# jankammeth/BA-path-planning

Measured on AMD Instinct MI355X. Metric: SCP iterations/sec (N agents x K waypoints), higher is better.
Workload: dtype f64

## Files before the change

ba-path-planning_amd/csrc/scp_kernels.hip:

```cpp
#include "scp_common.h"
#include "scp_pair_device.h"

#include <sys/prctl.h>
#include <time.h>

#include <atomic>
#include <chrono>
#include <cmath>
#include <cstdlib>
#include <map>
#include <mutex>
#include <type_traits>
#include <utility>

extern "C" int scp_abi_version(void) { return SCP_ABI_VERSION; }

extern "C" int scp_ctx_create(int device, void* hip_stream, scp_ctx** out) {
  if (!out) return SCP_ERR_INVALID;
  *out = nullptr;
  if (hipSetDevice(device) != hipSuccess) return SCP_ERR_HIP;
  scp_ctx* ctx = new scp_ctx();
  memset(ctx, 0, sizeof(*ctx));
  ctx->device = device;
  ctx->stream = (hipStream_t)hip_stream;
// ... 1511 lines not shown
  }
  __syncthreads();
  *total = tot;
  return base + incl - v;
}

__global__ __launch_bounds__(CMP_THREADS) void compact_count_kernel(const uint32_t* __restrict__ map, int64_t words,
                                                                     uint32_t* __restrict__ block_tot) {
  const int64_t w0 = (int64_t)blockIdx.x * CMP_WORDS + (int64_t)threadIdx.x * CMP_WPT;
  int c = 0;
#pragma unroll
  for (int i = 0; i < CMP_WPT; ++i)
    if (w0 + i < words) c += __popc(map[w0 + i]);
  int tot;
  block_exclusive_scan(c, &tot);
  if (threadIdx.x == 0) block_tot[blockIdx.x] = (uint32_t)tot;
}

__device__ inline void publish_stats(const scp_pair_stats* stats, unsigned long long n_selected, scp_stats_mirror* mirror,
                                     unsigned long long seq) {
  if (!mirror) return;
  const double mind = __hip_atomic_load(&stats->min_dist, __ATOMIC_RELAXED, __HIP_MEMORY_SCOPE_AGENT);
  const double maxv = __hip_atomic_load(&stats->max_violation, __ATOMIC_RELAXED, __HIP_MEMORY_SCOPE_AGENT);
  const unsigned long long fv =
      __hip_atomic_load((const unsigned long long*)&stats->first_violation, __ATOMIC_RELAXED, __HIP_MEMORY_SCOPE_AGENT);
  __hip_atomic_store((unsigned long long*)&mirror->stats.min_dist, (unsigned long long)__double_as_longlong(mind),
                     __ATOMIC_RELAXED, __HIP_MEMORY_SCOPE_SYSTEM);
  __hip_atomic_store((unsigned long long*)&mirror->stats.first_violation, fv, __ATOMIC_RELAXED, __HIP_MEMORY_SCOPE_SYSTEM);
  __hip_atomic_store((unsigned long long*)&mirror->stats.n_selected, n_selected, __ATOMIC_RELAXED, __HIP_MEMORY_SCOPE_SYSTEM);
  __hip_atomic_store((unsigned long long*)&mirror->stats.max_violation, (unsigned long long)__double_as_longlong(maxv),
                     __ATOMIC_RELAXED, __HIP_MEMORY_SCOPE_SYSTEM);
  __hip_atomic_store((unsigned long long*)&mirror->seq, seq, __ATOMIC_RELEASE, __HIP_MEMORY_SCOPE_SYSTEM);
}

__global__ __launch_bounds__(CMP_THREADS) void compact_scan_kernel(uint32_t* __restrict__ block_tot, int nblocks,
                                                                    scp_pair_stats* __restrict__ stats,
                                                                    scp_stats_mirror* __restrict__ mirror,
                                                                    unsigned long long seq) {
  int carry = 0;
  for (int b0 = 0; b0 < nblocks; b0 += CMP_THREADS) {
    const int b = b0 + threadIdx.x;
    const int v = b < nblocks ? (int)block_tot[b] : 0;
    int tot;
    const int ex = block_exclusive_scan(v, &tot);
    if (b < nblocks) block_tot[b] = (uint32_t)(carry + ex);
    carry += tot;
  }
  if (threadIdx.x == 0) {
    stats->n_selected = (unsigned long long)carry;
    publish_stats(stats, (unsigned long long)carry, mirror, seq);
  }
}

__global__ __launch_bounds__(CMP_THREADS) void compact_write_kernel(uint32_t* __restrict__ map, int64_t words,
                                                                     const uint32_t* __restrict__ block_off, int64_t nq,
                                                                     int64_t q_begin, int64_t pairs,
                                                                     int64_t* __restrict__ rows, int64_t cap,
                                                                     uint32_t* __restrict__ merge_into,
                                                                     const scp_pair_stats* __restrict__ stats) {
  const bool overflow = merge_into != nullptr && stats->n_selected > (unsigned long long)cap;
  const int64_t w0 = (int64_t)blockIdx.x * CMP_WORDS + (int64_t)threadIdx.x * CMP_WPT;
  uint32_t wd[CMP_WPT];
  int c = 0;
#pragma unroll
  for (int i = 0; i < CMP_WPT; ++i) {
    wd[i] = (w0 + i < words) ? map[w0 + i] : 0u;
    c += __popc(wd[i]);
  }
  int tot;
  int64_t slot = (int64_t)block_off[blockIdx.x] + block_exclusive_scan(c, &tot);
  if (tot == 0) return;
#pragma unroll
  for (int i = 0; i < CMP_WPT; ++i) {
    uint32_t m = wd[i];
    if (m && merge_into) {
      if (!overflow) merge_into[w0 + i] |= m;
      map[w0 + i] = 0u;
    }
    if (m) {
      const int64_t base = (w0 + i) * 32;
      const int64_t kk = base / nq, rr = base - kk * nq;
      while (m) {
        const int bit = __ffs((int)m) - 1;
        m &= m - 1;
        int64_t k2 = kk, r2 = rr + bit;
        while (r2 >= nq) {
          r2 -= nq;
          ++k2;
        }
        if (!overflow && slot < cap) rows[slot] = k2 * pairs + q_begin + r2;
        ++slot;
      }
    }
  }
}

constexpr int CMP1_THREADS = 1024;

template <int THREADS, bool COHERENT>
__device__ inline int compact_small_body(uint32_t* __restrict__ map, int64_t words, int64_t nq, int64_t q_begin,
                                         int64_t pairs, int64_t* __restrict__ rows, int64_t cap,
                                         uint32_t* __restrict__ merge_into, bool overwrite) {
  __shared__ int wsum[THREADS / 64];
  __shared__ int total_sh;
  constexpr int CHUNK = THREADS * CMP_WPT;
  const int lane = threadIdx.x & 63, wave = threadIdx.x >> 6;
  auto load = [&](int64_t w) -> uint32_t {
    return COHERENT ? __hip_atomic_load(map + w, __ATOMIC_RELAXED, __HIP_MEMORY_SCOPE_AGENT) : map[w];
  };
  int c_all = 0;
  for (int64_t w = threadIdx.x; w < words; w += THREADS) c_all += __popc(load(w));
#pragma unroll
  for (int o = 32; o > 0; o >>= 1) c_all += __shfl_xor(c_all, o);
  __syncthreads();
  if (lane == 0) wsum[wave] = c_all;
  __syncthreads();
  if (threadIdx.x == 0) {
    int t = 0;
    for (int w = 0; w < THREADS / 64; ++w) t += wsum[w];
    total_sh = t;
  }
  __syncthreads();
  const int total = total_sh;
// ... 61 lines not shown
__global__ __launch_bounds__(CMP1_THREADS) void compact_small_kernel(uint32_t* __restrict__ map, int64_t words, int64_t nq,
                                                                      int64_t q_begin, int64_t pairs,
                                                                      int64_t* __restrict__ rows, int64_t cap,
                                                                      uint32_t* __restrict__ merge_into,
                                                                      scp_pair_stats* __restrict__ stats,
                                                                      scp_stats_mirror* __restrict__ mirror,
                                                                      unsigned long long seq) {
  const int total = compact_small_body<CMP1_THREADS, false>(map, words, nq, q_begin, pairs, rows, cap, merge_into, false);
  if (threadIdx.x == 0) {
    stats->n_selected = (unsigned long long)total;
    publish_stats(stats, (unsigned long long)total, mirror, seq);
  }
}

static int ensure_cmp(scp_ctx* ctx, int64_t words) {
  const size_t need_map = (size_t)words * sizeof(uint32_t);
  const size_t need_tot = (size_t)(scp_cdiv(words, CMP_WORDS) + 1) * sizeof(uint32_t);
  if (ctx->cmp_map_bytes < need_map) {
    if (ctx->cmp_map) {
      SCP_HIP_CHECK(ctx, hipStreamSynchronize(ctx->stream));
      SCP_HIP_CHECK(ctx, hipFree(ctx->cmp_map));
      ctx->cmp_map = nullptr;
      ctx->cmp_map_bytes = 0;
    }
    SCP_HIP_CHECK(ctx, hipMalloc(&ctx->cmp_map, need_map));
    SCP_HIP_CHECK(ctx, hipMemsetAsync(ctx->cmp_map, 0, need_map, ctx->stream));
    ctx->cmp_map_bytes = need_map;
  }
  if (ctx->cmp_tot_bytes < need_tot) {
    if (ctx->cmp_tot) {
      SCP_HIP_CHECK(ctx, hipStreamSynchronize(ctx->stream));
      SCP_HIP_CHECK(ctx, hipFree(ctx->cmp_tot));
      ctx->cmp_tot = nullptr;
      ctx->cmp_tot_bytes = 0;
    }
    SCP_HIP_CHECK(ctx, hipMalloc(&ctx->cmp_tot, need_tot));
    ctx->cmp_tot_bytes = need_tot;
  }
  return SCP_OK;
}

static int launch_compaction(scp_ctx* ctx, uint32_t* map, int64_t words, int64_t nq, int64_t q_begin, int64_t pairs,
                             int64_t* rows, int64_t cap, uint32_t* merge_into, scp_pair_stats* stats) {
  if (words <= 0) return SCP_OK;
  const unsigned long long seq = ++ctx->mirror_seq;
  if (words <= CMP1_MAX_WORDS) {
    hipLaunchKernelGGL(compact_small_kernel, dim3(1), dim3(CMP1_THREADS), 0, ctx->stream, map, words, nq, q_begin, pairs,
                       rows, cap, merge_into, stats, ctx->d_mirror, seq);
    SCP_HIP_CHECK(ctx, hipGetLastError());
    return SCP_OK;
  }
  const int nblocks = scp_cdiv(words, CMP_WORDS);
  hipLaunchKernelGGL(compact_count_kernel, dim3(nblocks), dim3(CMP_THREADS), 0, ctx->stream, map, words, ctx->cmp_tot);
  hipLaunchKernelGGL(compact_scan_kernel, dim3(1), dim3(CMP_THREADS), 0, ctx->stream, ctx->cmp_tot, nblocks, stats,
                     ctx->d_mirror, seq);
  hipLaunchKernelGGL(compact_write_kernel, dim3(nblocks), dim3(CMP_THREADS), 0, ctx->stream, map, words, ctx->cmp_tot,
                     nq, q_begin, pairs, rows, cap, merge_into, stats);
  SCP_HIP_CHECK(ctx, hipGetLastError());
  return SCP_OK;
}

static int check_pair_range(scp_ctx* ctx, int N, int K, int D, int64_t q_begin, int64_t q_end) {
  SCP_REQUIRE(ctx, N >= 1 && K >= 1 && (D == 2 || D == 3), "pair pass: bad shape N=%d K=%d D=%d", N, K, D);
  SCP_REQUIRE(ctx, q_begin >= 0 && q_end >= q_begin && q_end <= scp_pairs(N),
              "pair pass: bad pair range [%lld, %lld) of %lld", (long long)q_begin, (long long)q_end,
              (long long)scp_pairs(N));
  SCP_REQUIRE(ctx, K <= 65535, "pair pass: K=%d exceeds grid.y", K);
  SCP_REQUIRE(ctx, q_end - q_begin < ((int64_t)1 << 31) - 2 * PAIR_ROWS,
              "pair pass: %lld pairs per call exceed the 32-bit lane offsets; shard the pair range",
              (long long)(q_end - q_begin));
  return SCP_OK;
}

int scp_check_pair_range(scp_ctx* ctx, int N, int K, int D, int64_t q_begin, int64_t q_end) {
  return check_pair_range(ctx, N, K, D, q_begin, q_end);
}

extern "C" int scp_linearize_pairs(scp_ctx* ctx, int N, int K, int D, double R, double h, int64_t q_begin,
                                   int64_t q_end, const double* pos_prev, const double* p0, const double* v0,
                                   double* eta_out, double* l_out, double margin, int64_t* sel_rows,
                                   int64_t sel_cap, uint32_t* sel_bitmap, scp_pair_stats* stats) {
  if (!ctx) return SCP_ERR_INVALID;
  int rc = check_pair_range(ctx, N, K, D, q_begin, q_end);
  if (rc) return rc;
  SCP_REQUIRE(ctx, pos_prev && p0 && v0 && eta_out && l_out && sel_bitmap && stats && (sel_rows || sel_cap == 0),
              "linearize_pairs: null pointer");
  SCP_REQUIRE(ctx, ((uintptr_t)eta_out % 16 == 0) && ((uintptr_t)l_out % 16 == 0),
              "linearize_pairs: eta/l must be 16-byte aligned");
  const int64_t nq = q_end - q_begin;
  PairArgs a{};
  a.N = N; a.K = K; a.D = D; a.R = R; a.h = h;
  a.q_begin = q_begin; a.q_end = q_end; a.pairs = scp_pairs(N);
  a.eta = eta_out; a.l = l_out; a.margin = margin;
  a.bitmap = sel_bitmap; a.mark = sel_bitmap; a.stats = stats;
  a.eta_stride = scp_eta_stride(K, nq);
  const int64_t words = (K * nq + 31) / 32;
  rc = ensure_cmp(ctx, words);
  if (rc) return rc;
  rc = launch_pair_pass<MODE_LINEARIZE>(ctx, a, pos_prev, p0, v0, sel_bitmap, words);
  if (rc) return rc;
  return launch_compaction(ctx, sel_bitmap, words, nq, q_begin, a.pairs, sel_rows, sel_cap, nullptr, stats);
}

extern "C" int scp_select_pairs(scp_ctx* ctx, int N, int K, int D, double R, int64_t q_begin, int64_t q_end,
                                const double* pos_prev, double margin, int64_t* sel_rows, int64_t sel_cap,
                                uint32_t* sel_bitmap, scp_pair_stats* stats) {
  if (!ctx) return SCP_ERR_INVALID;
  int rc = check_pair_range(ctx, N, K, D, q_begin, q_end);
  if (rc) return rc;
  SCP_REQUIRE(ctx, pos_prev && sel_bitmap && stats && (sel_rows || sel_cap == 0), "select_pairs: null pointer");
// ... 253 lines not shown
```

ba-path-planning_amd/csrc/scp_qp_fused.hip:

```cpp
#include "scp_qp_device.h"
#include "scp_pair_device.h"
#include "scp_reset_device.h"
#include <cstdlib>

namespace {

using namespace scpdev;
constexpr int FT = 1024;
constexpr int NWV = FT / 64;

#ifdef SCP_PHASE_PROFILE
__device__ unsigned long long scp_phase_clk[64];
#define PHASE_MARK(slot)                                                                      \
  do {                                                                                        \
    if (blockIdx.x == gridDim.x / 2 && threadIdx.x == 0) scp_phase_clk[slot] = wall_clock64(); \
  } while (0)
#else
#define PHASE_MARK(slot) ((void)0)
#endif

constexpr int SQ_BLOCKS = 128;
template <int E>
__global__ __launch_bounds__(FT) void cg1_col_kernel(int K, int Rf, int64_t C, double rho, double h,
                                                      const double* __restrict__ pMinv, const double* __restrict__ wrow,
// ... 539 lines not shown
        const int64_t g = (int64_t)row * C + col;
        const double zh = alpha * fma(a, v1[u], v0[u]) + (1.0 - alpha) * v2[u];
        const double y = v3[u];
        const double zn = fmin(fmax(zh + y / rr[u], v4[u]), v5[u]);
        const double yn = y + rr[u] * (zh - zn);
        yf[g] = yn;
        zf[g] = zn;
        Fx[g] = fma(aa, v1[u], v0[u]);
        if (dyf) dyf[g] = yn - y;
      } else if (row < rows) {
        const int64_t g = (int64_t)(row - Rf) * C + col;
        x[g] = fma(aa, v1[u], v0[u]);
        Qn[g] = fma(aa, v3[u], v2[u]);
      }
    }
    return;
  }
  const int64_t n = (int64_t)(blockIdx.x - eblocks) * 256 + threadIdx.x;
  const bool live = n < nW;
  double e[D], qi[D], qj[D], pi[D], pj[D], z = 0.0, y = 0.0, lo = 0.0;
  int posi = 0, posj = 0;
  if (live) {
    const int64_t bi = (int64_t)wk[n] * C + (int64_t)wi[n] * D;
    const int64_t bj = (int64_t)wk[n] * C + (int64_t)wj[n] * D;
#pragma unroll
    for (int d = 0; d < D; ++d) {
      e[d] = weta[n * D + d];
      qi[d] = Qx[bi + d]; qj[d] = Qx[bj + d]; pi[d] = Qp[bi + d]; pj[d] = Qp[bj + d];
    }
    z = zc[n]; y = yc[n]; lo = wl[n];
    posi = pos_i[n]; posj = pos_j[n];
  }
  const double a = inline_sq ? step_length_inline_256<D>(part_rz, npart, nW, C, rho_c, wk, wi, wj, weta, Qp)
                             : step_length_256(part_rz, npart, part_sq);
  const double aa = alpha * a;
  if (!live) return;
  double tc = 0.0, ax = 0.0;
#pragma unroll
  for (int d = 0; d < D; ++d) {
    tc += e[d] * (fma(a, pi[d], qi[d]) - fma(a, pj[d], qj[d]));
    ax += e[d] * (fma(aa, pi[d], qi[d]) - fma(aa, pj[d], qj[d]));
  }
  const double zh = alpha * tc + (1.0 - alpha) * z;
  const double zn = fmax(zh + y / rho_c, lo);
  const double yn = y + rho_c * (zh - zn);
  yc[n] = yn;
  zc[n] = zn;
  if (dyc) dyc[n] = fmin(yn - y, 0.0);
  const double g = (rho_c * zn - yn) - rho_c * ax;
  gval[posi] = g;
  gval[posj] = g;
}

template <int D, bool INIT>
__global__ __launch_bounds__(256) void rows_value_kernel(int64_t nW, int64_t C, double rho, const int* __restrict__ wk,
                                                          const int* __restrict__ wi, const int* __restrict__ wj,
                                                          const double* __restrict__ weta, const double* __restrict__ Q,
                                                          const double* __restrict__ zc, const double* __restrict__ yc,
                                                          const int* __restrict__ pos_i, const int* __restrict__ pos_j,
                                                          double* __restrict__ gval) {
  const int64_t n = (int64_t)blockIdx.x * 256 + threadIdx.x;
  if (n >= nW) return;
  const int64_t bi = (int64_t)wk[n] * C + (int64_t)wi[n] * D;
  const int64_t bj = (int64_t)wk[n] * C + (int64_t)wj[n] * D;
  double ax = 0.0;
#pragma unroll
  for (int d = 0; d < D; ++d) ax += weta[n * D + d] * (Q[bi + d] - Q[bj + d]);
  const double g = INIT ? (rho * zc[n] - yc[n]) - rho * ax : rho * ax;
  gval[pos_i[n]] = g;
  gval[pos_j[n]] = g;
}

#define FUSED_LAUNCHED(qp) SCP_HIP_CHECK((qp)->ctx, hipGetLastError())

template <typename Kern>
int allow_lds(scp_qp* qp, Kern kernel, size_t bytes) {
  if (bytes <= 64 * 1024) return SCP_OK;
  SCP_HIP_CHECK(qp->ctx, scp_raise_lds_limit(qp->ctx->device, reinterpret_cast<const void*>(kernel), bytes));
  return SCP_OK;
}

}

int scp_qp_qp0_iterations(scp_qp* qp, int nit, double* dy_out) {
  const QpDev& d = qp->d;
  hipStream_t s = qp->ctx->stream;
  const int K = qp->K, Rf = qp->Rf;
  const int64_t C = qp->C;
  const int nblk = (int)((C + CB - 1) / CB);
  const size_t lds = (size_t)CB * (pad_col(Rf) + 3 * pad_col(K)) * sizeof(double);
  if (K <= 64) {
    int rc = allow_lds(qp, qp0_col_kernel<1>, lds);
    if (rc) return rc;
    hipLaunchKernelGGL(qp0_col_kernel<1>, dim3(nblk), dim3(FT), lds, s, K, Rf, C, qp->rho, qp->st.sigma, qp->st.alpha, qp->h,
                       nit, d.pMinv, d.wrow, d.lf, d.uf, d.x, d.zf, d.yf, dy_out);
  } else {
    int rc = allow_lds(qp, qp0_col_kernel<2>, lds);
    if (rc) return rc;
    hipLaunchKernelGGL(qp0_col_kernel<2>, dim3(nblk), dim3(FT), lds, s, K, Rf, C, qp->rho, qp->st.sigma, qp->st.alpha, qp->h,
                       nit, d.pMinv, d.wrow, d.lf, d.uf, d.x, d.zf, d.yf, dy_out);
  }
  FUSED_LAUNCHED(qp);
  return SCP_OK;
}

namespace {
constexpr int CSR1_MAX_CELLS = 16384;
constexpr int64_t CSR1_MAX_ROWS = 1 << 18;
struct CsrNewRows {
  int64_t n, base;
  const int64_t* rows;
  const double *pos_prev, *p0, *v0;
  double R, h;
  int N;
  int64_t* w_row;
  double* wl;
};
__global__ void csr_small_kernel(int64_t nW, int K, int ncell, int D, int64_t C, double rho, int* __restrict__ wk,
                                 int* __restrict__ wi, int* __restrict__ wj, double* __restrict__ weta,
                                 const double* __restrict__ Qx, double* __restrict__ zc, double* __restrict__ yc,
                                 int* __restrict__ ptr, int* __restrict__ ent, double* __restrict__ coef,
                                 int* __restrict__ pos_i, int* __restrict__ pos_j, double* __restrict__ gval, CsrNewRows nr);
}

int scp_qp_cg1_prepare(scp_qp* qp) {
  if (qp->dv.carried) return SCP_OK;
  const QpDev& d = qp->d;
  hipStream_t s = qp->ctx->stream;
  const int K = qp->K;
  const int64_t C = qp->C;
  const double rho_c = qp->rho * qp->st.rho_col_scale;
  QP_CHECK(scp_qp_exact_qx(qp, true));
  const double* Qx = scp_qp_qx(qp);
  if (qp->dv.vals_rho_c == rho_c) {
  } else if (!qp->dv.lists && qp->nW > 0 && qp->nW <= CSR1_MAX_ROWS && qp->N * K <= CSR1_MAX_CELLS) {
    const int ncell = qp->N * K;
    hipLaunchKernelGGL(csr_small_kernel, dim3(1), dim3(1024), (size_t)ncell * sizeof(int), s, qp->nW, K, ncell, qp->D, C, rho_c,
                       d.w_k, d.w_i, d.w_j, d.w_eta, Qx, d.zc, d.yc, d.cell_ptr, d.ent_code, d.coef, d.pos_i, d.pos_j, d.gval,
                       CsrNewRows{});
    FUSED_LAUNCHED(qp);
  } else {
    QP_CHECK(scp_qp_csr_ensure(qp));
    const dim3 rgrid((unsigned)((qp->nW + 255) / 256)), rblock(256);
    if (qp->D == 2)
      hipLaunchKernelGGL((rows_value_kernel<2, true>), rgrid, rblock, 0, s, qp->nW, C, rho_c, d.w_k, d.w_i, d.w_j, d.w_eta, Qx,
                         d.zc, d.yc, d.pos_i, d.pos_j, d.gval);
    else
      hipLaunchKernelGGL((rows_value_kernel<3, true>), rgrid, rblock, 0, s, qp->nW, C, rho_c, d.w_k, d.w_i, d.w_j, d.w_eta, Qx,
                         d.zc, d.yc, d.pos_i, d.pos_j, d.gval);
    FUSED_LAUNCHED(qp);
  }
  qp_on_cg1_prepared(qp);
  return SCP_OK;
}

int scp_qp_install_rows_small(scp_qp* qp, int64_t n, const int64_t* rows, const double* pos_prev, const double* p0,
                              const double* v0, double R, const double* Qx, bool* done) {
  *done = false;
  const QpDev& d = qp->d;
  const int K = qp->K;
  const int64_t nW = qp->nW + n;
  if (!qp->dv.qx || n <= 0 || nW > CSR1_MAX_ROWS || qp->N * K > CSR1_MAX_CELLS) return SCP_OK;
  const int ncell = qp->N * K;
  const double rho_c = qp->rho * qp->st.rho_col_scale;
  CsrNewRows nr{n, qp->nW, rows, pos_prev, p0, v0, R, qp->h, qp->N, d.w_row, d.w_l};
  hipLaunchKernelGGL(csr_small_kernel, dim3(1), dim3(1024), (size_t)ncell * sizeof(int), qp->ctx->stream, nW, K, ncell, qp->D,
                     qp->C, rho_c, d.w_k, d.w_i, d.w_j, d.w_eta, Qx, d.zc, d.yc, d.cell_ptr, d.ent_code, d.coef, d.pos_i,
                     d.pos_j, d.gval, nr);
  FUSED_LAUNCHED(qp);
  *done = true;
  return SCP_OK;
}

int scp_qp_cg1_iteration(scp_qp* qp, int* cg_count, bool emit_dy) {
  const QpDev& d = qp->d;
  double* dyf = emit_dy ? d.dyf : nullptr;
  double* dyc = emit_dy ? d.dyc : nullptr;
  hipStream_t s = qp->ctx->stream;
  const int K = qp->K, Rf = qp->Rf;
  const int64_t C = qp->C;
  const int nblk = (int)((C + CB - 1) / CB);
  double* Qp = d.s0p;
  double* Fp = d.tf;
  double* part_rz = d.part;
  double* part_sq = d.part + SCP_PART_CAP / 2;
  const double rho_c = qp->rho * qp->st.rho_col_scale;
  QP_CHECK(scp_qp_cg1_prepare(qp));
  double* Qx = scp_qp_qx(qp);
  double* Qn = scp_qp_qx(qp, true);
  const size_t lds = (size_t)CB * (pad_col(Rf) + 5 * pad_col(K)) * sizeof(double);
  int npart = nblk;
  if (K > SCP_FUSED_MAX_K) {
    npart = (int)C;
// ... 88 lines not shown

__global__ __launch_bounds__(256) void csr_scan_add_kernel(int ncell, int nblk, int* __restrict__ ptr, int* __restrict__ cur,
                                                            const int* __restrict__ blk_tot) {
  int off = 0;
  for (int b = 0; b < (int)blockIdx.x; ++b) off += blk_tot[b];
  const int c = blockIdx.x * SCAN_CELLS + SCAN_SC * (int)threadIdx.x;
#pragma unroll
  for (int e = 0; e < SCAN_SC; ++e) {
    if (c + e < ncell) {
      const int v = ptr[c + e] + off;
      ptr[c + e] = v;
      cur[c + e] = v;
    }
  }
  if (blockIdx.x == nblk - 1 && threadIdx.x == 0) ptr[ncell] = off + blk_tot[nblk - 1];
}

__global__ __launch_bounds__(256) void csr_fill_kernel(int64_t nW, int K, const int* __restrict__ wk,
                                                        const int* __restrict__ wi, const int* __restrict__ wj,
                                                        int* __restrict__ cur, int* __restrict__ ent) {
  const int64_t n = (int64_t)blockIdx.x * 256 + threadIdx.x;
  if (n >= nW) return;
  ent[atomicAdd(cur + cell_of(wk[n], wi[n], K), 1)] = (int)(2 * n);
  ent[atomicAdd(cur + cell_of(wk[n], wj[n], K), 1)] = (int)(2 * n + 1);
}

__global__ __launch_bounds__(256) void csr_sort_kernel(int ncell, const int* __restrict__ ptr, int* __restrict__ ent) {
  const int c = blockIdx.x * 256 + threadIdx.x;
  if (c >= ncell) return;
  const int b = ptr[c], e = ptr[c + 1];
  for (int i = b + 1; i < e; ++i) {
    const int v = ent[i];
    int j = i - 1;
    while (j >= b && ent[j] > v) {
      ent[j + 1] = ent[j];
      --j;
    }
    ent[j + 1] = v;
  }
}

__global__ __launch_bounds__(256) void csr_finish_kernel(int64_t nent, int D, const int* __restrict__ ent,
                                                          const double* __restrict__ weta, double* __restrict__ coef,
                                                          int* __restrict__ pos_i, int* __restrict__ pos_j) {
  const int64_t t = (int64_t)blockIdx.x * 256 + threadIdx.x;
  if (t >= nent) return;
  const int code = ent[t];
  const int n = code >> 1, side = code & 1;
  for (int d = 0; d < D; ++d) coef[t * D + d] = side ? -weta[(int64_t)n * D + d] : weta[(int64_t)n * D + d];
  if (side) pos_j[n] = (int)t;
  else pos_i[n] = (int)t;
}

template <bool COH>
__device__ inline void csr_small_body(int* csr_cnt, int64_t nW, int K, int ncell, int D, int64_t C, double rho,
                                                          int* __restrict__ wk, int* __restrict__ wi,
                                                          int* __restrict__ wj, double* __restrict__ weta,
                                                          const double* __restrict__ Qx, double* __restrict__ zc,
                                                          double* __restrict__ yc, int* __restrict__ ptr,
                                                          int* __restrict__ ent, double* __restrict__ coef,
                                                          int* __restrict__ pos_i, int* __restrict__ pos_j,
                                                          double* __restrict__ gval, CsrNewRows nr) {
  __shared__ int wsum[16];
  constexpr int SC = CSR1_MAX_CELLS / 1024;
  const int tid = threadIdx.x, lane = tid & 63, wave = tid >> 6;
  if (nr.n > 0) {
    const int64_t pairs = (int64_t)nr.N * (nr.N - 1) / 2;
    for (int64_t t = tid; t < nr.n; t += 1024) {
      if (D == 2)
        add_row_at<2, COH>(t, nr.N, K, C, pairs, nr.base, nr.rows, nr.pos_prev, nr.p0, nr.v0, nr.R, nr.h, Qx, nr.w_row, wk, wi, wj,
                      weta, nr.wl, zc, yc);
      else
        add_row_at<3, COH>(t, nr.N, K, C, pairs, nr.base, nr.rows, nr.pos_prev, nr.p0, nr.v0, nr.R, nr.h, Qx, nr.w_row, wk, wi, wj,
                      weta, nr.wl, zc, yc);
    }
    __threadfence_block();
    __syncthreads();
  }
  for (int c = tid; c < ncell; c += 1024) csr_cnt[c] = 0;
  __syncthreads();
  for (int64_t n = tid; n < nW; n += 1024) {
    atomicAdd(&csr_cnt[cell_of(wk[n], wi[n], K)], 1);
    atomicAdd(&csr_cnt[cell_of(wk[n], wj[n], K)], 1);
  }
  __syncthreads();
  {
    int v[SC], tot = 0;
#pragma unroll
    for (int e = 0; e < SC; ++e) {
      v[e] = SC * tid + e < ncell ? csr_cnt[SC * tid + e] : 0;
      tot += v[e];
    }
    int incl = tot;
#pragma unroll
    for (int o = 1; o < 64; o <<= 1) {
      const int t = __shfl_up(incl, o);
      if (lane >= o) incl += t;
    }
    if (lane == 63) wsum[wave] = incl;
    __syncthreads();
    int run = incl - tot;
    for (int w = 0; w < wave; ++w) run += wsum[w];
#pragma unroll
    for (int e = 0; e < SC; ++e) {
      if (SC * tid + e < ncell) {
        csr_cnt[SC * tid + e] = run;
// ... 88 lines not shown
                               const double* p0, const double* v0, double R, double* Qx, bool* done) {
  *done = false;
  const QpDev& d = qp->d;
  const int K = qp->K;
  if (n <= 0 || n > CSR1_MAX_ROWS || qp->N * K > CSR1_MAX_CELLS) return SCP_OK;
  const int ncell = qp->N * K;
  const double rho_c = qp->rho * qp->st.rho_col_scale;
  const size_t lds = std::max((size_t)K * RESET_COLS * sizeof(double), (size_t)ncell * sizeof(int));
  CsrNewRows nr{n, 0, rows, pos_prev, p0, v0, R, qp->h, qp->N, d.w_row, d.w_l};
  ResetArgs ra{qp->N, qp->Rf, x0, d.F, d.S0, d.x, d.zf, d.fx, d.yf};
  hipLaunchKernelGGL(reset_install_kernel, dim3((unsigned)scp_cdiv(qp->C, RESET_COLS)), dim3(1024), lds, qp->ctx->stream, ra, n,
                     K, ncell, qp->D, qp->C, rho_c, d.w_k, d.w_i, d.w_j, d.w_eta, Qx, d.zc, d.yc, d.cell_ptr, d.ent_code,
                     d.coef, d.pos_i, d.pos_j, d.gval, nr, qp->ctx->d_ticket + 2);
  FUSED_LAUNCHED(qp);
  *done = true;
  return SCP_OK;
}

namespace {
__global__ __launch_bounds__(256) void csr_rowval_kernel(int64_t nW, int mode, double rho, const double* __restrict__ zc,
                                                          const double* __restrict__ yc, const double* __restrict__ vec,
                                                          const int* __restrict__ pos_i, const int* __restrict__ pos_j,
                                                          double* __restrict__ gval, const double* __restrict__ vec2,
                                                          double* __restrict__ gval2) {
  const int64_t n = (int64_t)blockIdx.x * 256 + threadIdx.x;
  if (n >= nW) return;
  if (gval2) {
    const double g2 = vec2[n];
    gval2[pos_i[n]] = g2;
    gval2[pos_j[n]] = g2;
  }
  const double g = mode == 0 ? rho * zc[n] - yc[n] : (mode == 1 ? yc[n] : vec[n]);
  gval[pos_i[n]] = g;
  gval[pos_j[n]] = g;
}

__global__ __launch_bounds__(256) void csr_gather_kernel(int K, int N, int D, const int* __restrict__ ptr,
                                                          const double* __restrict__ coef,
                                                          const double* __restrict__ gval, double* __restrict__ G) {
  const int64_t t = (int64_t)blockIdx.x * 256 + threadIdx.x;
  const int64_t C = (int64_t)N * D;
  if (t >= C * K) return;
  const int k = (int)(t / C), col = (int)(t % C);
  const int agent = col / D, d = col - agent * D;
  const int cell = cell_of(k, agent, K);
  double acc = 0.0;
  const int t1 = ptr[cell + 1];
  for (int e = ptr[cell]; e < t1; ++e) acc += coef[(size_t)e * D + d] * gval[e];
  G[t] = acc;
}

}

int scp_qp_csr_ensure(scp_qp* qp) {
  if (qp->dv.lists) return SCP_OK;
  const QpDev& d = qp->d;
  hipStream_t s = qp->ctx->stream;
  const int ncell = qp->N * qp->K;
  SCP_REQUIRE(qp->ctx, 2 * qp->nW < 0x3FFFFFFF, "csr_build: too many working rows for 32-bit entry codes");
  SCP_HIP_CHECK(qp->ctx, hipMemsetAsync(d.cell_ptr, 0, (size_t)(ncell + 1) * sizeof(int), s));
  if (qp->nW > 0) {
    const dim3 rgrid((unsigned)((qp->nW + 255) / 256));
    hipLaunchKernelGGL(csr_count_kernel, rgrid, dim3(256), 0, s, qp->nW, qp->K, d.w_k, d.w_i, d.w_j, d.cell_ptr);
    const int sblk = (ncell + SCAN_CELLS - 1) / SCAN_CELLS;
    hipLaunchKernelGGL(csr_scan_local_kernel, dim3(sblk), dim3(256), 0, s, ncell, d.cell_ptr, d.scan_tot);
    hipLaunchKernelGGL(csr_scan_add_kernel, dim3(sblk), dim3(256), 0, s, ncell, sblk, d.cell_ptr, d.cell_cur, d.scan_tot);
    hipLaunchKernelGGL(csr_fill_kernel, rgrid, dim3(256), 0, s, qp->nW, qp->K, d.w_k, d.w_i, d.w_j, d.cell_cur, d.ent_code);
    hipLaunchKernelGGL(csr_sort_kernel, dim3((ncell + 255) / 256), dim3(256), 0, s, ncell, d.cell_ptr, d.ent_code);
    hipLaunchKernelGGL(csr_finish_kernel, dim3((unsigned)((2 * qp->nW + 255) / 256)), dim3(256), 0, s, 2 * qp->nW, qp->D,
                       d.ent_code, d.w_eta, d.coef, d.pos_i, d.pos_j);
    FUSED_LAUNCHED(qp);
  }
  qp_on_lists_built(qp);
  return SCP_OK;
}

int scp_qp_csr_scatter(scp_qp* qp, int mode, const double* vec) {
  QP_CHECK(scp_qp_csr_ensure(qp));
  const QpDev& d = qp->d;
  hipStream_t s = qp->ctx->stream;
  const int64_t nx = (int64_t)qp->K * qp->C;
  hipLaunchKernelGGL(csr_rowval_kernel, dim3((unsigned)((qp->nW + 255) / 256)), dim3(256), 0, s, qp->nW, mode,
                     qp->rho * qp->st.rho_col_scale, d.zc, d.yc, vec, d.pos_i, d.pos_j, d.gval, (const double*)nullptr, (double*)nullptr);
  hipLaunchKernelGGL(csr_gather_kernel, dim3((unsigned)((nx + 255) / 256)), dim3(256), 0, s, qp->K, qp->N, qp->D,
                     d.cell_ptr, d.coef, d.gval, d.G);
  FUSED_LAUNCHED(qp);
  return SCP_OK;
}

int scp_qp_rows_gather(scp_qp* qp, const double* Q) {
  const QpDev& d = qp->d;
  hipStream_t s = qp->ctx->stream;
  QP_CHECK(scp_qp_csr_ensure(qp));
  const int64_t C = qp->C, nx = (int64_t)qp->K * C;
  const double rho_c = qp->rho * qp->st.rho_col_scale;
  const dim3 rgrid((unsigned)((qp->nW + 255) / 256)), rblock(256);
  if (qp->D == 2)
    hipLaunchKernelGGL((rows_value_kernel<2, false>), rgrid, rblock, 0, s, qp->nW, C, rho_c, d.w_k, d.w_i, d.w_j, d.w_eta, Q,
                       d.zc, d.yc, d.pos_i, d.pos_j, d.gval);
  else
    hipLaunchKernelGGL((rows_value_kernel<3, false>), rgrid, rblock, 0, s, qp->nW, C, rho_c, d.w_k, d.w_i, d.w_j, d.w_eta, Q,
                       d.zc, d.yc, d.pos_i, d.pos_j, d.gval);
  hipLaunchKernelGGL(csr_gather_kernel, dim3((unsigned)((nx + 255) / 256)), dim3(256), 0, s, qp->K, qp->N, qp->D,
                     d.cell_ptr, d.coef, d.gval, d.G);
  FUSED_LAUNCHED(qp);
  return SCP_OK;
}

namespace {
struct PackDesc {
  const double* src;
  double* dst;
  int R, M;
};
struct PackArgs {
  PackDesc m[2];
};
__global__ __launch_bounds__(256) void pack_operands_kernel(PackArgs a) {
  const PackDesc d = a.m[blockIdx.y];
  const int nks = (d.M + 3) >> 2;
// ... 328 lines not shown
```

ba-path-planning_amd/csrc/scp_qp_internal.h:

```cpp
#pragma once
#include "scp_common.h"

constexpr int SCP_KKT_SLOTS = 6;
constexpr int SCP_KKT_SLOTS_MAX = 32;
constexpr size_t SCP_KKT_POOL_BYTES = (size_t)48 << 20;
constexpr int NPART = 128;

#define QP_CHECK(call)            \
  do {                            \
    int rc_ = (call);             \
    if (rc_ != SCP_OK) return rc_; \
  } while (0)

enum Slot {
  SL_RZ0 = 0, SL_RZ1 = 1,
  SL_RP = 8, SL_NAX = 9, SL_NZ = 10, SL_RD = 11, SL_NPX = 12, SL_NATY = 13,
  SL_NDY = 14, SL_SUPP = 15, SL_NATDY = 16,
  SL_COUNT = 32
};

struct QpDev {
  double *F, *Ft, *S0, *S0t, *HS, *Hf, *Minv, *aug, *wrow;
  double* gj_tmp;
  double* G0;
  double* pMinv;
  double *T, *pT;
  double *lf, *uf, *zf, *yf, *wf, *tf;
  double* states;
  double *x, *xt, *rhs, *r, *p, *zz, *G;
  double* HQ;
  int64_t* w_row;
  int *w_k, *w_i, *w_j;
  double *w_eta, *w_l, *zc, *yc;
  double* scal;
  double* part;
  double* s0p;
  double* fx;
  double* dyf;
  double* dyc;
  int* cell_ptr;
  int* cell_cur;
  int* scan_tot;
  int* ent_code;
  double* coef;
  double* gval;
  double* gval2;
  double* gval3;
  int *pos_i, *pos_j;
  double* kkt_pool;
  unsigned long long* sync_words;
  unsigned long long* cells;
  unsigned long long* gpart;
  unsigned long long* gcheck;
};

struct QpDerived {
  bool lists = false;
  bool qx = false;
  int qx_half = 0;
  double vals_rho_c = 0.0;
  bool carried = false;
};

struct scp_qp {
  scp_ctx* ctx;
  int N, K, D, Rf;
  int64_t C;
  double h;
  scp_qp_settings st;
  int64_t row_cap, nW;
  bool problem_set, reset_done;
  QpDerived dv;
  double rho;
  QpDev d;
  struct KktSlot {
    double rho, sigma;
    unsigned long long used;
    double *Hf, *HS, *Minv, *T, *pMinv, *pT;
  } kkt[SCP_KKT_SLOTS_MAX];
  int n_kkt;
  unsigned long long kkt_clock;
  double* h_scal;
  double* h_scal_dev;
  unsigned long long check_seq;
  double space[6];
  double lim[6];
  int64_t steps_since_reset;
  int persist_variant;
  int persist_fault;
  bool persist_off;
  bool persist_skip_solve;
  int persist_gave_up_total;
  int64_t persist_cap_nW;
  int persist_cap;
  unsigned long long persist_epoch;
  unsigned* h_persist;
  int persist_rho_switches;
  double persist_rho;
  unsigned* h_persist_dev;
};

constexpr int64_t SCP_FINE_MAX_COLUMNS = 4096;
inline int scp_qp_fine_cadence(const scp_qp* qp) {
  const scp_qp_settings& st = qp->st;
  const bool fine = st.check_fine > 0 && st.check_fine < st.check_termination && st.check_termination % st.check_fine == 0 &&
                    qp->nW > 0 && qp->C <= SCP_FINE_MAX_COLUMNS;
  return fine ? st.check_fine : 0;
}

constexpr int SCP_RESID_STRIDE = 12;
constexpr int SCP_RESID_CAP = (4096 / 2 + 128) * SCP_RESID_STRIDE;
constexpr int SCP_INV_LDS_MAX_K = 96;
constexpr int SCP_BIGK_MAX_K = 1024;
constexpr int SCP_FUSED_MAX_K = 120;
constexpr int SCP_PART_CAP = 4096;
int scp_qp_cg1_iteration(scp_qp* qp, int* cg_count, bool emit_dy);
int scp_qp_qp0_iterations(scp_qp* qp, int nit, double* dy_out);
int scp_qp_csr_scatter(scp_qp* qp, int mode, const double* vec);
int scp_qp_csr_ensure(scp_qp* qp);
int scp_qp_rows_gather(scp_qp* qp, const double* Q);
int scp_qp_cg1_prepare(scp_qp* qp);
int scp_qp_exact_qx(scp_qp* qp, bool with_fx);
inline double* scp_qp_qx(const scp_qp* qp, bool other = false) {
  return (qp->dv.qx_half != 0) != other ? qp->d.HQ : qp->d.HQ + (int64_t)qp->K * qp->C;
}
// ... 39 lines not shown
```

Measured before the change: 414.1.

## Fold compaction scan into write kernel and fuse CSR build with row values

For small passes, the compaction write kernel now computes its own block offset and the total selected count by reducing the per-block counts itself, which removes the separate single-block scan launch. The CSR build for the small-pass path is restructured into count, single-pass scan, fill-down with atomics, and a per-cell sort that also writes coef, pos and the initial row values. This drops the separate finish and rows_value launches. The aim is fewer kernel launches on a launch-latency-bound path, at the cost of redundant reads of the block totals by every block and a serial insertion sort per cell.

```diff
diff --git a/ba-path-planning_amd/csrc/scp_kernels.hip b/ba-path-planning_amd/csrc/scp_kernels.hip
--- a/ba-path-planning_amd/csrc/scp_kernels.hip
+++ b/ba-path-planning_amd/csrc/scp_kernels.hip
@@ -1587,13 +1587,52 @@
   }
 }
 
+template <bool SCAN>
 __global__ __launch_bounds__(CMP_THREADS) void compact_write_kernel(uint32_t* __restrict__ map, int64_t words,
                                                                      const uint32_t* __restrict__ block_off, int64_t nq,
                                                                      int64_t q_begin, int64_t pairs,
                                                                      int64_t* __restrict__ rows, int64_t cap,
                                                                      uint32_t* __restrict__ merge_into,
-                                                                     const scp_pair_stats* __restrict__ stats) {
-  const bool overflow = merge_into != nullptr && stats->n_selected > (unsigned long long)cap;
+                                                                     scp_pair_stats* __restrict__ stats,
+                                                                     scp_stats_mirror* __restrict__ mirror,
+                                                                     unsigned long long seq) {
+  unsigned long long n_selected;
+  int64_t my_off;
+  if (SCAN) {
+    __shared__ int sum_sh[2][CMP_THREADS / 64];
+    int before = 0, all = 0;
+    for (int b = threadIdx.x; b < (int)gridDim.x; b += CMP_THREADS) {
+      const int v = (int)block_off[b];
+      all += v;
+      if (b < (int)blockIdx.x) before += v;
+    }
+#pragma unroll
+    for (int o = 32; o > 0; o >>= 1) {
+      before += __shfl_xor(before, o);
+      all += __shfl_xor(all, o);
+    }
+    if ((threadIdx.x & 63) == 0) {
+      sum_sh[0][threadIdx.x >> 6] = before;
+      sum_sh[1][threadIdx.x >> 6] = all;
+    }
+    __syncthreads();
+    before = all = 0;
+#pragma unroll
+    for (int w = 0; w < CMP_THREADS / 64; ++w) {
+      before += sum_sh[0][w];
+      all += sum_sh[1][w];
+    }
+    n_selected = (unsigned long long)all;
+    my_off = before;
+    if (blockIdx.x == 0 && threadIdx.x == 0) {
+      stats->n_selected = n_selected;
+      publish_stats(stats, n_selected, mirror, seq);
+    }
+  } else {
+    n_selected = stats->n_selected;
+    my_off = (int64_t)block_off[blockIdx.x];
+  }
+  const bool overflow = merge_into != nullptr && n_selected > (unsigned long long)cap;
   const int64_t w0 = (int64_t)blockIdx.x * CMP_WORDS + (int64_t)threadIdx.x * CMP_WPT;
   uint32_t wd[CMP_WPT];
   int c = 0;
@@ -1603,7 +1642,7 @@
     c += __popc(wd[i]);
   }
   int tot;
-  int64_t slot = (int64_t)block_off[blockIdx.x] + block_exclusive_scan(c, &tot);
+  int64_t slot = my_off + block_exclusive_scan(c, &tot);
   if (tot == 0) return;
 #pragma unroll
   for (int i = 0; i < CMP_WPT; ++i) {
@@ -1771,10 +1810,15 @@
   }
   const int nblocks = scp_cdiv(words, CMP_WORDS);
   hipLaunchKernelGGL(compact_count_kernel, dim3(nblocks), dim3(CMP_THREADS), 0, ctx->stream, map, words, ctx->cmp_tot);
-  hipLaunchKernelGGL(compact_scan_kernel, dim3(1), dim3(CMP_THREADS), 0, ctx->stream, ctx->cmp_tot, nblocks, stats,
-                     ctx->d_mirror, seq);
-  hipLaunchKernelGGL(compact_write_kernel, dim3(nblocks), dim3(CMP_THREADS), 0, ctx->stream, map, words, ctx->cmp_tot,
-                     nq, q_begin, pairs, rows, cap, merge_into, stats);
+  if (ctx->small_pass) {
+    hipLaunchKernelGGL(compact_write_kernel<true>, dim3(nblocks), dim3(CMP_THREADS), 0, ctx->stream, map, words, ctx->cmp_tot,
+                       nq, q_begin, pairs, rows, cap, merge_into, stats, ctx->d_mirror, seq);
+  } else {
+    hipLaunchKernelGGL(compact_scan_kernel, dim3(1), dim3(CMP_THREADS), 0, ctx->stream, ctx->cmp_tot, nblocks, stats,
+                       ctx->d_mirror, seq);
+    hipLaunchKernelGGL(compact_write_kernel<false>, dim3(nblocks), dim3(CMP_THREADS), 0, ctx->stream, map, words, ctx->cmp_tot,
+                       nq, q_begin, pairs, rows, cap, merge_into, stats, (scp_stats_mirror*)nullptr, 0ULL);
+  }
   SCP_HIP_CHECK(ctx, hipGetLastError());
   return SCP_OK;
 }
diff --git a/ba-path-planning_amd/csrc/scp_qp_fused.hip b/ba-path-planning_amd/csrc/scp_qp_fused.hip
--- a/ba-path-planning_amd/csrc/scp_qp_fused.hip
+++ b/ba-path-planning_amd/csrc/scp_qp_fused.hip
@@ -615,6 +615,18 @@
   gval[posj] = g;
 }
 
+template <int D>
+__device__ inline double row_value_init(int64_t n, int64_t C, double rho, const int* __restrict__ wk, const int* __restrict__ wi,
+                                        const int* __restrict__ wj, const double* __restrict__ weta, const double* __restrict__ Q,
+                                        const double* __restrict__ zc, const double* __restrict__ yc) {
+  const int64_t bi = (int64_t)wk[n] * C + (int64_t)wi[n] * D;
+  const int64_t bj = (int64_t)wk[n] * C + (int64_t)wj[n] * D;
+  double ax = 0.0;
+#pragma unroll
+  for (int d = 0; d < D; ++d) ax += weta[n * D + d] * (Q[bi + d] - Q[bj + d]);
+  return (rho * zc[n] - yc[n]) - rho * ax;
+}
+
 template <int D, bool INIT>
 __global__ __launch_bounds__(256) void rows_value_kernel(int64_t nW, int64_t C, double rho, const int* __restrict__ wk,
                                                           const int* __restrict__ wi, const int* __restrict__ wj,
@@ -624,12 +636,17 @@
                                                           double* __restrict__ gval) {
   const int64_t n = (int64_t)blockIdx.x * 256 + threadIdx.x;
   if (n >= nW) return;
-  const int64_t bi = (int64_t)wk[n] * C + (int64_t)wi[n] * D;
-  const int64_t bj = (int64_t)wk[n] * C + (int64_t)wj[n] * D;
-  double ax = 0.0;
-#pragma unroll
-  for (int d = 0; d < D; ++d) ax += weta[n * D + d] * (Q[bi + d] - Q[bj + d]);
-  const double g = INIT ? (rho * zc[n] - yc[n]) - rho * ax : rho * ax;
+  double g;
+  if (INIT) {
+    g = row_value_init<D>(n, C, rho, wk, wi, wj, weta, Q, zc, yc);
+  } else {
+    const int64_t bi = (int64_t)wk[n] * C + (int64_t)wi[n] * D;
+    const int64_t bj = (int64_t)wk[n] * C + (int64_t)wj[n] * D;
+    double ax = 0.0;
+#pragma unroll
+    for (int d = 0; d < D; ++d) ax += weta[n * D + d] * (Q[bi + d] - Q[bj + d]);
+    g = rho * ax;
+  }
   gval[pos_i[n]] = g;
   gval[pos_j[n]] = g;
 }
@@ -686,6 +703,8 @@
                                  int* __restrict__ pos_i, int* __restrict__ pos_j, double* __restrict__ gval, CsrNewRows nr);
 }
 
+static int csr_build_with_values(scp_qp* qp, double rho_c, const double* Qx);
+
 int scp_qp_cg1_prepare(scp_qp* qp) {
   if (qp->dv.carried) return SCP_OK;
   const QpDev& d = qp->d;
@@ -702,6 +721,8 @@
                        d.w_k, d.w_i, d.w_j, d.w_eta, Qx, d.zc, d.yc, d.cell_ptr, d.ent_code, d.coef, d.pos_i, d.pos_j, d.gval,
                        CsrNewRows{});
     FUSED_LAUNCHED(qp);
+  } else if (!qp->dv.lists && qp->nW > 0 && qp->ctx->small_pass) {
+    QP_CHECK(csr_build_with_values(qp, rho_c, Qx));
   } else {
     QP_CHECK(scp_qp_csr_ensure(qp));
     const dim3 rgrid((unsigned)((qp->nW + 255) / 256)), rblock(256);
@@ -896,6 +917,86 @@
   else pos_i[n] = (int)t;
 }
 
+__global__ __launch_bounds__(256) void csr_scan_kernel(int ncell, const int* __restrict__ cnt, int* __restrict__ ptr) {
+  __shared__ int wsum[4], wpre[4];
+  const int lane = threadIdx.x & 63, wave = threadIdx.x >> 6;
+  const int c0 = blockIdx.x * SCAN_CELLS;
+  int pre = 0;
+  for (int q = threadIdx.x; q < c0 / 4; q += 256) {
+    const int4 w = reinterpret_cast<const int4*>(cnt)[q];
+    pre += (w.x + w.y) + (w.z + w.w);
+  }
+#pragma unroll
+  for (int o = 32; o > 0; o >>= 1) pre += __shfl_xor(pre, o);
+  const int c = c0 + SCAN_SC * (int)threadIdx.x;
+  int v[SCAN_SC], tot = 0;
+#pragma unroll
+  for (int e = 0; e < SCAN_SC; ++e) {
+    v[e] = c + e < ncell ? cnt[c + e] : 0;
+    tot += v[e];
+  }
+  int incl = tot;
+  incl += dpp_mov0_i32<0x111, 0xF>(incl);
+  incl += dpp_mov0_i32<0x112, 0xF>(incl);
+  incl += dpp_mov0_i32<0x114, 0xF>(incl);
+  incl += dpp_mov0_i32<0x118, 0xF>(incl);
+  incl += dpp_mov0_i32<0x142, 0xA>(incl);
+  incl += dpp_mov0_i32<0x143, 0xC>(incl);
+  if (lane == 63) wsum[wave] = incl;
+  if (lane == 0) wpre[wave] = pre;
+  __syncthreads();
+  int run = incl - tot + ((wpre[0] + wpre[1]) + (wpre[2] + wpre[3]));
+  for (int w = 0; w < wave; ++w) run += wsum[w];
+#pragma unroll
+  for (int e = 0; e < SCAN_SC; ++e) {
+    if (c + e < ncell) ptr[c + e] = run;
+    run += v[e];
+  }
+  if (blockIdx.x == gridDim.x - 1 && threadIdx.x == 255) ptr[ncell] = run;
+}
+
+__global__ __launch_bounds__(256) void csr_fill_down_kernel(int64_t nW, int K, const int* __restrict__ wk,
+                                                             const int* __restrict__ wi, const int* __restrict__ wj,
+                                                             const int* __restrict__ ptr, int* __restrict__ cnt,
+                                                             int* __restrict__ ent) {
+  const int64_t n = (int64_t)blockIdx.x * 256 + threadIdx.x;
+  if (n >= nW) return;
+  const int ci = cell_of(wk[n], wi[n], K), cj = cell_of(wk[n], wj[n], K);
+  ent[ptr[ci] + atomicSub(cnt + ci, 1) - 1] = (int)(2 * n);
+  ent[ptr[cj] + atomicSub(cnt + cj, 1) - 1] = (int)(2 * n + 1);
+}
+
+template <int D>
+__global__ __launch_bounds__(256) void csr_cells_kernel(int ncell, int64_t C, double rho, const int* __restrict__ ptr,
+                                                         int* __restrict__ ent, const int* __restrict__ wk,
+                                                         const int* __restrict__ wi, const int* __restrict__ wj,
+                                                         const double* __restrict__ weta, const double* __restrict__ Qx,
+                                                         const double* __restrict__ zc, const double* __restrict__ yc,
+                                                         double* __restrict__ coef, int* __restrict__ pos_i,
+                                                         int* __restrict__ pos_j, double* __restrict__ gval) {
+  const int c = blockIdx.x * 256 + threadIdx.x;
+  if (c >= ncell) return;
+  const int b = ptr[c], e = ptr[c + 1];
+  for (int i = b + 1; i < e; ++i) {
+    const int v = ent[i];
+    int j = i - 1;
+    while (j >= b && ent[j] > v) {
+      ent[j + 1] = ent[j];
+      --j;
+    }
+    ent[j + 1] = v;
+  }
+  for (int t = b; t < e; ++t) {
+    const int code = ent[t];
+    const int n = code >> 1, side = code & 1;
+#pragma unroll
+    for (int d = 0; d < D; ++d) coef[(int64_t)t * D + d] = side ? -weta[(int64_t)n * D + d] : weta[(int64_t)n * D + d];
+    if (side) pos_j[n] = t;
+    else pos_i[n] = t;
+    gval[t] = row_value_init<D>(n, C, rho, wk, wi, wj, weta, Qx, zc, yc);
+  }
+}
+
 template <bool COH>
 __device__ inline void csr_small_body(int* csr_cnt, int64_t nW, int K, int ncell, int D, int64_t C, double rho,
                                                           int* __restrict__ wk, int* __restrict__ wi,
@@ -1090,6 +1191,31 @@
 
 }
 
+static int csr_build_with_values(scp_qp* qp, double rho_c, const double* Qx) {
+  const QpDev& d = qp->d;
+  hipStream_t s = qp->ctx->stream;
+  const int ncell = qp->N * qp->K;
+  SCP_REQUIRE(qp->ctx, 2 * qp->nW < 0x3FFFFFFF, "csr_build: too many working rows for 32-bit entry codes");
+  if (!qp->csr_cnt_zero) {
+    SCP_HIP_CHECK(qp->ctx, hipMemsetAsync(d.cell_cur, 0, (size_t)ncell * sizeof(int), s));
+    qp->csr_cnt_zero = true;
+  }
+  const dim3 rgrid((unsigned)((qp->nW + 255) / 256)), cgrid((unsigned)((ncell + 255) / 256));
+  hipLaunchKernelGGL(csr_count_kernel, rgrid, dim3(256), 0, s, qp->nW, qp->K, d.w_k, d.w_i, d.w_j, d.cell_cur);
+  hipLaunchKernelGGL(csr_scan_kernel, dim3((ncell + SCAN_CELLS - 1) / SCAN_CELLS), dim3(256), 0, s, ncell, d.cell_cur, d.cell_ptr);
+  hipLaunchKernelGGL(csr_fill_down_kernel, rgrid, dim3(256), 0, s, qp->nW, qp->K, d.w_k, d.w_i, d.w_j, d.cell_ptr, d.cell_cur,
+                     d.ent_code);
+  if (qp->D == 2)
+    hipLaunchKernelGGL(csr_cells_kernel<2>, cgrid, dim3(256), 0, s, ncell, qp->C, rho_c, d.cell_ptr, d.ent_code, d.w_k, d.w_i,
+                       d.w_j, d.w_eta, Qx, d.zc, d.yc, d.coef, d.pos_i, d.pos_j, d.gval);
+  else
+    hipLaunchKernelGGL(csr_cells_kernel<3>, cgrid, dim3(256), 0, s, ncell, qp->C, rho_c, d.cell_ptr, d.ent_code, d.w_k, d.w_i,
+                       d.w_j, d.w_eta, Qx, d.zc, d.yc, d.coef, d.pos_i, d.pos_j, d.gval);
+  FUSED_LAUNCHED(qp);
+  qp_on_lists_built(qp);
+  return SCP_OK;
+}
+
 int scp_qp_csr_ensure(scp_qp* qp) {
   if (qp->dv.lists) return SCP_OK;
   const QpDev& d = qp->d;
@@ -1104,6 +1230,7 @@
     hipLaunchKernelGGL(csr_scan_local_kernel, dim3(sblk), dim3(256), 0, s, ncell, d.cell_ptr, d.scan_tot);
     hipLaunchKernelGGL(csr_scan_add_kernel, dim3(sblk), dim3(256), 0, s, ncell, sblk, d.cell_ptr, d.cell_cur, d.scan_tot);
     hipLaunchKernelGGL(csr_fill_kernel, rgrid, dim3(256), 0, s, qp->nW, qp->K, d.w_k, d.w_i, d.w_j, d.cell_cur, d.ent_code);
+    qp->csr_cnt_zero = false;
     hipLaunchKernelGGL(csr_sort_kernel, dim3((ncell + 255) / 256), dim3(256), 0, s, ncell, d.cell_ptr, d.ent_code);
     hipLaunchKernelGGL(csr_finish_kernel, dim3((unsigned)((2 * qp->nW + 255) / 256)), dim3(256), 0, s, 2 * qp->nW, qp->D,
                        d.ent_code, d.w_eta, d.coef, d.pos_i, d.pos_j);
diff --git a/ba-path-planning_amd/csrc/scp_qp_internal.h b/ba-path-planning_amd/csrc/scp_qp_internal.h
--- a/ba-path-planning_amd/csrc/scp_qp_internal.h
+++ b/ba-path-planning_amd/csrc/scp_qp_internal.h
@@ -71,6 +71,7 @@
   int64_t row_cap, nW;
   bool problem_set, reset_done;
   QpDerived dv;
+  bool csr_cnt_zero;
   double rho;
   QpDev d;
   struct KktSlot {
```

New measurement: 418.6, median of 6. About the same (+1.1%).
